# OnurBasci/TransformerBasedNavierStokeSolver

Hardware: AMD Instinct MI355X
Metric: ns64_train_samples_per_s (higher is better)
Workload: dtype f32

## Files before the change

transformerbasednavierstokesolver_amd/csrc/pa2d_gemm.hip:

```cpp
#include "pa2d_gemm_common.h"
#include <string.h>


static Pa2dEnv read_env() {
    auto is = [](const char* n, const char* pre) { const char* e = getenv(n); return e && strncmp(e, pre, strlen(pre)) == 0; };
    auto num = [](const char* n, int dflt) { const char* e = getenv(n); return (e && e[0]) ? atoi(e) : dflt; };
    Pa2dEnv v;
    v.conv_halo = is("PA2D_CONV_HALO", "o") ? 0 : (is("PA2D_CONV_HALO", "f") ? 2 : 1);
    v.mc_big_off = is("PA2D_MC_BIG", "o") ? 1 : 0;
    v.kc_bk16 = num("PA2D_KC_BK", 0) == 16 ? 1 : 0;
    v.mc_bk = num("PA2D_MC_BK", 16) == 32 ? 32 : 16;
    v.mc_splits = num("PA2D_MC_SPLITS", 0);
    v.mcb_splits = num("PA2D_MCB_SPLITS", 0);
    v.lin_dw_split = is("PA2D_LIN_DW_SPLIT", "of") ? 0 : 1;
    v.lin_panel = is("PA2D_LIN_PANEL", "of") ? 0 : 1;
    v.lin_rowpanel = is("PA2D_LIN_ROWPANEL", "of") ? 0 : 1;
    v.lin_small_split = is("PA2D_LIN_SMALL_SPLIT", "of") ? 0 : 1;
    v.conv_mfma16 = num("PA2D_CONV_MFMA", 16) == 32 ? 0 : 1;
    v.mc_mfma16 = num("PA2D_MC_MFMA", 16) == 32 ? 0 : 1;
    v.split_big = num("PA2D_SPLIT_BIG", 1);
    v.slice_map = is("PA2D_SLICE_MAP", "l") ? 0 : 1;
    v.default_engine = is("PA2D_GEMM", "f") ? 0 : (is("PA2D_GEMM", "b") ? 2 : 1);
    return v;
}
static Pa2dEnv g_env = read_env();
const Pa2dEnv& pa2d_env() { return g_env; }
static int kc_bk(bool im2col, int Cin) {
    if (im2col && pa2d_env().kc_bk16) return 16;
    return (!im2col || (Cin % 32) == 0) ? 32 : 16;
}
KCTile kc_tile(int M, int N, bool im2col, int Cin) {
    const int tiles_m = ceil_div(M, 128);
    const long long t128 = (long long)tiles_m * ceil_div(N, 128);
    const long long t12864 = (long long)tiles_m * ceil_div(N, 64);
    const int bk = kc_bk(im2col, Cin);
    if (N > 64 && t128 >= 384) return {128, 128, bk};
    if (t12864 >= 384 || M <= 64) return {128, 64, bk};
// ... 169 lines not shown

int pa2d_gemm_bwd_data(const float* dy, long long lddy, const float* w, long long ldw, const float* pre,
                       long long ldpre, int act, float* dx, long long lddx, const void* wimg, void* ws, size_t ws_bytes, int M,
                       int N, int K, int engine, hipStream_t st) {
    if (ldw != K) return PA2D_ERR_ARG;
    if (N & 3) return PA2D_ERR_ARG;
    if (M <= 0) return PA2D_OK;
    if (ws_bytes < (size_t)N * K * sizeof(float)) return PA2D_ERR_WORKSPACE;
    float* const wt_ws = (float*)ws;
    KCParams p = dense_bwd_data_params(dy, lddy, wt_ws, pre, ldpre, act, dx, lddx, M, N, K, engine, false);
    const size_t img = rowpanel_image_bytes(K, N, engine);
    if (img && wimg) p.wimg = const_cast<void*>(wimg);
    else if (img && ws_bytes >= (size_t)N * K * sizeof(float) + img) {
        p.wimg = (char*)ws + (size_t)N * K * sizeof(float); p.wsrc = w; p.wsn = 1; p.wsk = ldw;
    }
    if (!(p.wimg && rowpanel_applies(p) && (M % 128) == 0)) {
        const int rc = launch_repack(w, nullptr, wt_ws, 0, N, K, 0, 0, st);
        if (rc) return rc;
    }
    return launch_kc(p, false, st);
}

size_t pa2d_gemm_bwd_weight_workspace(int M, int N, int K, int engine) {
    (void)engine;
    const MCPlan pl = plan_mc(N, K, M);
    return (pl.slab_floats + (size_t)pl.splits * N) * sizeof(float);
}

int pa2d_gemm_bwd_weight(const float* dy, long long lddy, const float* x, long long ldx, float* dw, float* db,
                         void* ws, size_t ws_bytes, int M, int N, int K, int accumulate, int engine, hipStream_t st) {
    if (!engine_ok(engine)) return PA2D_ERR_ARG;
    if (M <= 0) {
        if (accumulate) return PA2D_OK;
        const int rz = pa2d_zero(dw, sizeof(float) * N * K, st);
        return rz ? rz : pa2d_zero(db, sizeof(float) * N, st);
    }
    if (ws_bytes < pa2d_gemm_bwd_weight_workspace(M, N, K, engine)) return PA2D_ERR_WORKSPACE;
    const MCPlan pl = plan_mc(N, K, M);
    float* cs = db ? (float*)ws + pl.slab_floats : nullptr;
    const bool bfk = (engine == 1 || engine == 2) && pl.big && mc_f32src_applies(N, K, M, lddy, ldx);
    int rc = bfk ? launch_mc_f32src(dy, lddy, N, x, ldx, K, M, (float*)ws, pl, engine == 2 ? 1 : 3, cs, st)
                 : launch_mc(dy, lddy, N, x, ldx, K, M, false, 0, 0, 0, (float*)ws, pl, engine, st, cs);
    if (rc) return rc;
    rc = launch_reduce((const float*)ws, pl.splits, (long long)N * K, dw, nullptr, 0, 0, 0, st, accumulate);
    if (rc) return rc;
    if (db) rc = launch_reduce(cs, pl.splits, N, db, nullptr, 0, 0, 0, st, accumulate);
    return rc;
}


int pa2d_gemm_bias_act_fwd_bf16(const void* x, long long ldx, const float* w, long long ldw, const float* bias,
                                const void* res, long long ldres, void* y, long long ldy, void* pre, long long ldpre,
                                int M, int N, int K, int act, hipStream_t st) {
    return launch_kc(dense_fwd_params(x, ldx, w, ldw, bias, res, ldres, y, ldy, pre, ldpre, M, N, K, act, 2, true), false, st);
}

int pa2d_gemm_bwd_data_bf16(const void* dy, long long lddy, const float* w, long long ldw, const void* pre,
                            long long ldpre, int act, void* dx, long long lddx, float* wt_ws, int M, int N, int K,
                            hipStream_t st) {
    if (ldw != K) return PA2D_ERR_ARG;
    if (N & 3) return PA2D_ERR_ARG;
    if (M <= 0) return PA2D_OK;
    int rc = launch_repack(w, nullptr, wt_ws, 0, N, K, 0, 0, st);
    if (rc) return rc;
    return launch_kc(dense_bwd_data_params(dy, lddy, wt_ws, pre, ldpre, act, dx, lddx, M, N, K, 2, true), false, st);
}

size_t pa2d_gemm_bwd_weight_workspace_bf16(int M, int N, int K) {
    const MCPlan pl = plan_mc_planes_big(N, K, M);
    size_t a = pl.slab_floats, b = (size_t)colsum_blocks(M) * N;
// ... 24 lines not shown
```

transformerbasednavierstokesolver_amd/csrc/pa2d_gemm_common.h:

```cpp
#pragma once
#include "pa2d_internal.h"
#include "pa2d_bf16_split.h"
#include <stdlib.h>

#define EPI_ACT 1
#define EPI_STORE_PRE 2
#define EPI_MUL_DACT 4

struct KCParams {
    const float* A; long long lda;
    const float* B; long long ldb;
    float* C; long long ldc;
    const float* bias;
    const float* bias2; int bias_split;
    int depth;
    const float* res; long long ldres;
    float* aux; long long ldaux;
    int M, N, K;
    int act, epi;
    int H, W, Cin;
    unsigned a_bytes, b_bytes;
    unsigned c_bytes, res_bytes, aux_bytes;
    int apre;
    int engine;
// ... 69 lines not shown
    } else if (p.epi == EPI_ACT && gelu && !has_res) {
        KC_EPI(false, false, true, false, ACT_GELU)
    } else if (p.epi == EPI_MUL_DACT && gelu && !has_res) {
        KC_EPI(false, false, false, true, ACT_GELU)
    } else {
        const bool sp = p.epi & EPI_STORE_PRE, ac = p.epi & EPI_ACT, da = p.epi & EPI_MUL_DACT;
        if (da) { if (has_res) { KC_EPI(true, false, false, true, -1) } else { KC_EPI(false, false, false, true, -1) } }
        else if (sp && ac) { if (has_res) { KC_EPI(true, true, true, false, -1) } else { KC_EPI(false, true, true, false, -1) } }
        else if (ac) { if (has_res) { KC_EPI(true, false, true, false, -1) } else { KC_EPI(false, false, true, false, -1) } }
        else { if (has_res) { KC_EPI(true, true, false, false, -1) } else { KC_EPI(false, true, false, false, -1) } }
    }
#undef KC_EPI
}

struct MCParams {
    const float* A; long long lda; int Mi;
    int depth;
    const float* B; long long ldb; int Nj;
    float* slab;
    int Mk, chunks_per_split, splits;
    int H, W, Cin;
    unsigned a_bytes, b_bytes;
    float* colsum;
};
struct MCPlan { int big; int splits; int chunks_per_split; size_t slab_floats; };
struct KCTile { int bm, bn, bk; };

static inline bool engine_ok(int e) { return e >= 0 && e <= 2; }
bool use_split(int engine, int N, bool im2col, int Cin);
KCTile kc_tile(int M, int N, bool im2col, int Cin);
int launch_kc(const KCParams& p_in, bool im2col, hipStream_t st, hipEvent_t ev0 = nullptr, hipEvent_t ev1 = nullptr);
int launch_repack(const float* w0, const float* w1, float* dst, int mode, int N, int K, int C, int Cin, hipStream_t st,
                  int taps = 9);
int launch_kc_f32(const KCParams& p, bool im2col, const KCTile& t, hipStream_t st);
int launch_kc_split(KCParams& p, bool im2col, hipStream_t st);
bool kc_split_small_applies(const KCParams& p, bool im2col);
int launch_kc_split_small(const KCParams& p, hipStream_t st);
size_t planes_bytes(long long rows, int C, int NT);
int launch_split_planes(const float* src, long long ld, void* dst, long long rows, int C, int NT, hipStream_t st);
int launch_repack_split(const float* w0, const float* w1, void* dst, int bwd, int NT, int C, int Cin, hipStream_t st,
                        int taps = 9);
bool panel_applies(const KCParams& p, bool im2col);
int launch_kc_panel(const KCParams& p, hipStream_t st);
size_t rowpanel_image_bytes(int N, int K, int engine);
bool rowpanel_applies(const KCParams& p);
int launch_pack_weight_image(const float* w, long long sn, long long sk, void* img, int N, int K, hipStream_t st);
int launch_kc_rowpanel(const KCParams& p, const void* img, hipStream_t st);
bool conv_halo_applies(const KCParams& p);
int launch_conv_halo(const KCParams& p, hipStream_t st);
MCPlan plan_mc(int Mi, int Nj, int Mk);
int launch_mc(const float* A, long long lda, int Mi, const float* B, long long ldb, int Nj, int Mk, bool im2col,
              int H, int W, int Cin, float* slab, const MCPlan& pl, int engine, hipStream_t st, float* colsum = nullptr,
              int taps = 9, int depth = 1);
int launch_reduce(const float* slab, int nslab, long long count, float* out, float* out2, int mode, int C, int Cin,
                  hipStream_t st, int accumulate = 0, int taps = 9);
int pa2d_launch_reduce(const float* slab, int nslab, long long count, float* out, hipStream_t st);
bool mc_planes_supported(int C, int Cin);
int launch_mc_planes(const void* PA, const void* PB, int C, int Cin, int Mk, int H, int W, float* slab,
                     const MCPlan& pl, int NT, hipStream_t st);
bool mc_planes_big_applies(int C, int Cin, int Mk);
MCPlan plan_mc_planes_big(int Mi, int Nj, int Mk);
int launch_mc_planes_big(const void* PA, const void* PB, int C, int Cin, int Mk, int H, int W, float* slab,
                         const MCPlan& pl, int NT, hipStream_t st);
int launch_mc_planes_big_raw(const void* PA, int Mi, const void* PB, int Cin, int taps, int Mk, int H, int W, float* slab,
                             const MCPlan& pl, int NT, hipStream_t st);
bool mc_f32src_applies(int Mi, int Nj, int Mk, long long lda, long long ldb);
int launch_mc_f32src(const float* A, long long lda, int Mi, const float* B, long long ldb, int Nj, int Mk, float* slab,
                     const MCPlan& pl, int NT, float* colsum, hipStream_t st);
int colsum_blocks(int M);
int launch_colsum_bf16(const void* X, long long ld, int M, int N, float* out, float* partial, hipStream_t st,
                       float* out2 = nullptr, int split = 0, int accumulate = 0);
int launch_colsum(const float* X, long long ld, int M, int N, float* out, float* partial, hipStream_t st,
                  float* out2 = nullptr, int split = 0, int accumulate = 0);
```

transformerbasednavierstokesolver_amd/csrc/pa2d_gemm_mc.hip:

```cpp
#include "pa2d_gemm_common.h"


template <int NT>
__device__ __forceinline__ void mc_split_elem(float v, bf16x8 (&pl)[NT], int e) {
    const __bf16 h = (__bf16)v;
    pl[0][e] = h;
    if constexpr (NT == 3) {
        const float r1 = v - (float)h;
        const __bf16 m = (__bf16)r1;
        pl[1][e] = m;
        pl[2][e] = (__bf16)(r1 - (float)m);
    }
}
template <int BM, int BN, bool IM2COL, int NT, int BK = 16, int TAPS = 9>
__global__ __launch_bounds__(256, 2) void gemm_mc_kernel(const MCParams p) {
    constexpr int WM = BM / 2, WN = BN / 2, TM = WM / 32, TN = WN / 32;
    constexpr int A_TPR = BM / 4, A_RPP = 256 / A_TPR, A_IT = BK / A_RPP;
    constexpr int B_TPR = BN / 4, B_RPP = 256 / B_TPR, B_IT = BK / B_RPP;
    static_assert(TM >= 1 && TN >= 1 && A_IT >= 1 && B_IT >= 1, "tile");
    __shared__ __attribute__((aligned(16))) float smem[2 * BK * (BM + BN)];
    float* const As = smem;
    float* const Bs = smem + 2 * BK * BM;

    const int tid = threadIdx.x, lane = tid & 63, wave = tid >> 6;
// ... 148 lines not shown
                    acc[i][j] = __builtin_amdgcn_mfma_f32_32x32x2f32(af[kk & 1][i], bf[kk & 1][j], acc[i][j], 0, 0, 0);
        }
        __builtin_amdgcn_sched_group_barrier(0x100, TM + TN, 0);
#pragma unroll
        for (int kk = 0; kk < BK / 2 - 1; ++kk) {
            __builtin_amdgcn_sched_group_barrier(0x100, TM + TN, 0);
            __builtin_amdgcn_sched_group_barrier(0x008, TM * TN, 0);
        }
        __builtin_amdgcn_sched_group_barrier(0x008, TM * TN, 0);
        }
        if (c + 1 < c_end) MC_STORE(buf ^ 1)
        __syncthreads();
    }
#undef MC_LOAD
#undef MC_STORE

    if (do_cs) {
        *reinterpret_cast<float4*>(smem + a_r * BM + a_c) = cs;
        __syncthreads();
        for (int c = tid; c < BM; c += 256) {
            float t = 0.f;
#pragma unroll
            for (int r = 0; r < A_RPP; ++r) t += smem[r * BM + c];
            if (ti * BM + c < p.Mi) p.colsum[(size_t)split * p.Mi + ti * BM + c] = t;
        }
    }
    float* out = p.slab + (size_t)split * p.Mi * p.Nj;
    const int col0 = tj * BN + wn * WN + (lane & 31);
    const int row0 = ti * BM + wm * WM + 4 * (lane >> 5);
#pragma unroll
    for (int j = 0; j < TN; ++j) {
        const int col = col0 + j * 32;
        if (col >= p.Nj) continue;
#pragma unroll
        for (int i = 0; i < TM; ++i)
#pragma unroll
            for (int r = 0; r < 16; ++r) {
                const int row = row0 + i * 32 + (r & 3) + 8 * (r >> 2);
                if (row < p.Mi) out[(size_t)row * p.Nj + col] = acc[i][j][r];
            }
    }
}


MCPlan plan_mc(int Mi, int Nj, int Mk) {
    MCPlan pl;
    if (Mk < 1) Mk = 1;
    pl.big = (Mi > 64 && Nj > 64) ? 1 : 0;
    const int bm = pl.big ? 128 : 64;
    const int tiles = ceil_div(Mi, bm) * ceil_div(Nj, bm);
// ... 39 lines not shown
        }
        for (; k < nslab; k += 4) s0 += p[(size_t)k * count];
    }
    red[ty][tx] = (s0 + s1) + (s2 + s3);
    __syncthreads();
    if (ty != 0 || idx >= count) return;
    const float s = ((red[0][tx] + red[1][tx]) + red[2][tx]) + red[3][tx];
    float* dst;
    if (mode == 0) {
        dst = out + idx;
    } else if (mode == 2) {
        dst = idx < C ? out + idx : out2 + (idx - C);
    } else {
        const int ci = (int)(idx % Cin);
        const int tap = (int)((idx / Cin) % TAPS);
        const int co = (int)(idx / ((long long)Cin * TAPS));
        dst = (co < C ? out : out2) + ((size_t)(co % C) * Cin + ci) * TAPS + tap;
    }
    *dst = accumulate ? *dst + s : s;
}

int launch_mc(const float* A, long long lda, int Mi, const float* B, long long ldb, int Nj, int Mk,
                     bool im2col, int H, int W, int Cin, float* slab, const MCPlan& pl, int engine, hipStream_t st,
                     float* colsum, int taps, int depth) {
    if ((Mi & 3) || (Nj & 3) || (lda & 3) || (ldb & 3)) return PA2D_ERR_ARG;
    if (im2col && (Cin & 3)) return PA2D_ERR_UNSUPPORTED;
    MCParams p;
    p.A = A; p.lda = lda; p.Mi = Mi; p.B = B; p.ldb = ldb; p.Nj = Nj; p.slab = slab; p.Mk = Mk;
    p.chunks_per_split = pl.chunks_per_split; p.splits = pl.splits; p.H = H; p.W = W; p.Cin = Cin;
    p.colsum = colsum;
    p.depth = depth;
    {
        const unsigned long long ab = ((unsigned long long)(Mk - 1) * lda + Mi) * 4ull;
        const unsigned long long bb = ((unsigned long long)(Mk - 1) * ldb + (im2col ? Cin : Nj)) * 4ull;
        if (ab >= 0xFFFFFFF0ull || bb >= 0xFFFFFFF0ull) return PA2D_ERR_UNSUPPORTED;
        p.a_bytes = (unsigned)ab;
        p.b_bytes = (unsigned)bb;
    }
    const int bm = pl.big ? 128 : 64;
    const dim3 grid(ceil_div(Mi, bm) * ceil_div(Nj, bm) * pl.splits);
    const bool bf = engine == 2;
    const int mc_bk = pa2d_env().mc_bk;
    if (im2col && taps == 27) {
        if (pl.big && !bf && mc_bk == 32 && (pl.chunks_per_split % 2) == 0)
            hipLaunchKernelGGL((gemm_mc_kernel<128, 128, true, 0, 32, 27>), grid, dim3(256), 0, st, p);
        else if (pl.big && engine == 1 && (Cin % 32) == 0)
            hipLaunchKernelGGL((gemm_mc_kernel<128, 128, true, 3, 16, 27>), grid, dim3(256), 0, st, p);
        else if (pl.big && bf)
            hipLaunchKernelGGL((gemm_mc_kernel<128, 128, true, 1, 16, 27>), grid, dim3(256), 0, st, p);
        else if (pl.big)
            hipLaunchKernelGGL((gemm_mc_kernel<128, 128, true, 0, 16, 27>), grid, dim3(256), 0, st, p);
        else
            hipLaunchKernelGGL((gemm_mc_kernel<64, 64, true, 0, 16, 27>), grid, dim3(256), 0, st, p);
        PA2D_CHECK_LAUNCH();
// ... 126 lines not shown
```

transformerbasednavierstokesolver_amd/csrc/pa2d_gemm_mc_planes.hip:

```cpp
#include "pa2d_gemm_common.h"
#include "pa2d_bf16_split.h"

struct MCPlanesParams {
    const void* PA; int chA;
    const void* PB; int chB;
    float* slab;
    int Mi, Nj, Mk, chunks_per_split, splits, H, W, Cin;
    unsigned a_bytes, b_bytes;
    int taps;
    long long lda, ldb;
    float* colsum;
};

__device__ __forceinline__ unsigned img_off(int row, int ch) {
    return 256u * row + 16u * (ch ^ (((row & 3) << 2) | ((row >> 2) & 3)));
}

template <int NT, int KS, bool F32SRC = false, bool MF16 = false>
__global__ __launch_bounds__(256, 2) void gemm_mc_planes_kernel(const MCPlanesParams p) {
    constexpr int PIMG = 4096;
    constexpr int STAGE = 2 * NT * KS * PIMG;
    constexpr int NP = 2 * NT * KS;
    __shared__ __attribute__((aligned(16))) unsigned char smem[(MF16 ? 3 : 2) * STAGE];

    const int tid = threadIdx.x, lane = tid & 63, wave = tid >> 6;
    const int tiles_i = (p.Mi + 127) / 128, tiles_j = (p.Nj + 127) / 128;
    int tj, ti, split;
    {
        const int tiles = tiles_i * tiles_j;
        if ((p.splits & 7) == 0) {
            const int xcd = blockIdx.x & 7, slot = blockIdx.x >> 3, q = p.splits >> 3;
            split = xcd * q + slot / tiles;
            const int t = slot % tiles;
            tj = t % tiles_j;
// ... 192 lines not shown
                MP16_MMA(ib, afc)
#pragma unroll
                for (int pl = 0; pl < NT; ++pl) afc[pl] = afn[pl];
            }
            __syncthreads();
            const int t = sp;
            sp = sr;
            sr = sq;
            sq = t;
        }
#undef MP16_CONVERT
#undef MP16_WRITE
#undef MP16_MMA
#undef MP16_FRAG
        if (do_cs) {
            float* sm = reinterpret_cast<float*>(smem);
#pragma unroll
            for (int e = 0; e < 8; ++e) sm[frow * 128 + fc8 * 8 + e] = cs[e];
            __syncthreads();
            if (tid < 128) {
                float t = 0.f;
#pragma unroll
                for (int r = 0; r < 16; ++r) t += sm[r * 128 + tid];
                if (ti * 128 + tid < p.Mi) p.colsum[(size_t)split * p.Mi + ti * 128 + tid] = t;
            }
        }
        float* out = p.slab + (size_t)split * p.Mi * p.Nj;
#pragma unroll
        for (int j = 0; j < 4; ++j) {
            const int col = tj * 128 + wn * 64 + j * 16 + 4 * kq;
#pragma unroll
            for (int ib = 0; ib < 4; ++ib) {
                const int row = ti * 128 + wm * 64 + ib * 16 + (lane & 15);
                if (row < p.Mi && col < p.Nj) *reinterpret_cast<f32x4*>(out + (size_t)row * p.Nj + col) = acc[ib][j];
            }
        }
        return;
    }

    f32x16 acc[2][2];
#pragma unroll
    for (int i = 0; i < 2; ++i)
#pragma unroll
        for (int j = 0; j < 2; ++j)
#pragma unroll
            for (int r = 0; r < 16; ++r) acc[i][j][r] = 0.f;

    const int g = lane >> 4, q4 = (lane & 15) >> 2, pq = lane & 3;
    unsigned fa[2][2], fb[2][2];
#pragma unroll
// ... 43 lines not shown
                    acc[i][j] = __builtin_amdgcn_mfma_f32_32x32x16_bf16(af[i][0], bf[j][2], acc[i][j], 0, 0, 0);
                    acc[i][j] = __builtin_amdgcn_mfma_f32_32x32x16_bf16(af[i][1], bf[j][0], acc[i][j], 0, 0, 0);
                    acc[i][j] = __builtin_amdgcn_mfma_f32_32x32x16_bf16(af[i][0], bf[j][1], acc[i][j], 0, 0, 0);
                }
                acc[i][j] = __builtin_amdgcn_mfma_f32_32x32x16_bf16(af[i][0], bf[j][0], acc[i][j], 0, 0, 0);
            }
        }
        if (c + KS < c_end) { MP_STORE(buf ^ 1) }
        __syncthreads();
    }
#undef MP_LOAD
#undef MP_STORE

    if constexpr (F32SRC) {
        if (do_cs) {
            float* sm = reinterpret_cast<float*>(smem);
#pragma unroll
            for (int e = 0; e < 8; ++e) sm[frow * 128 + fc8 * 8 + e] = cs[e];
            __syncthreads();
            if (tid < 128) {
                float t = 0.f;
#pragma unroll
                for (int r = 0; r < 16; ++r) t += sm[r * 128 + tid];
                if (ti * 128 + tid < p.Mi) p.colsum[(size_t)split * p.Mi + ti * 128 + tid] = t;
            }
        }
    }
    float* out = p.slab + (size_t)split * p.Mi * p.Nj;
    const int col0 = tj * 128 + wn * 64 + (lane & 31);
    const int row0 = ti * 128 + wm * 64 + 4 * (lane >> 5);
#pragma unroll
    for (int j = 0; j < 2; ++j)
#pragma unroll
        for (int i = 0; i < 2; ++i)
#pragma unroll
            for (int r = 0; r < 16; ++r) {
                const int row = row0 + i * 32 + (r & 3) + 8 * (r >> 2);
                if (!F32SRC || (row < p.Mi && col0 + j * 32 < p.Nj)) out[(size_t)row * p.Nj + col0 + j * 32] = acc[i][j][r];
            }
}

bool mc_planes_supported(int C, int Cin) { return (C % 64) == 0 && (Cin % 128) == 0; }

int launch_mc_planes(const void* PA, const void* PB, int C, int Cin, int Mk, int H, int W, float* slab,
                     const MCPlan& pl, int NT, hipStream_t st) {
    if (!mc_planes_supported(C, Cin) || !pl.big) return PA2D_ERR_UNSUPPORTED;
    MCPlanesParams p;
    p.PA = PA; p.chA = 2 * C / 32; p.PB = PB; p.chB = Cin / 32; p.slab = slab;
    p.Mi = 2 * C; p.Nj = 9 * Cin; p.Mk = Mk; p.chunks_per_split = pl.chunks_per_split; p.splits = pl.splits;
    p.H = H; p.W = W; p.Cin = Cin; p.taps = 9;
    const unsigned long long ab = (unsigned long long)Mk * p.chA * NT * 64, bb = (unsigned long long)Mk * p.chB * NT * 64;
    if (ab >= 0xFFFFFFF0ull || bb >= 0xFFFFFFF0ull) return PA2D_ERR_UNSUPPORTED;
    p.a_bytes = (unsigned)ab; p.b_bytes = (unsigned)bb;
    const dim3 grid((p.Mi / 128) * (p.Nj / 128) * pl.splits);
    if (NT == 3) hipLaunchKernelGGL((gemm_mc_planes_kernel<3, 1>), grid, dim3(256), 0, st, p);
    else hipLaunchKernelGGL((gemm_mc_planes_kernel<1, 4>), grid, dim3(256), 0, st, p);
    PA2D_CHECK_LAUNCH();
    return PA2D_OK;
}

template <int NT, int KS, bool MF16 = false>
__global__ __launch_bounds__(512, 1) void gemm_mc_planes_big_kernel(const MCPlanesParams p, const int per_xcd) {
    constexpr int PIMG = 8192;
    constexpr int STAGE = 2 * NT * KS * PIMG;
    constexpr int NP = (2 * NT * KS * 512) / 512;
    extern __shared__ __attribute__((aligned(16))) unsigned char smem[];

    const int tid = threadIdx.x, lane = tid & 63, wave = tid >> 6;
    const int tiles_i = (p.Mi + 255) / 256, tiles_j = (p.Nj + 255) / 256;
    const int tiles = tiles_i * tiles_j;
    const int lin = (blockIdx.x & 7) * per_xcd + (blockIdx.x >> 3);
    if ((int)(blockIdx.x >> 3) >= per_xcd || lin >= tiles * p.splits) return;
    const int split = lin / tiles, t_ = lin - split * tiles;
    const int ti = t_ / tiles_j, tj = t_ - ti * tiles_j;
    const int wm = wave >> 2, wn = wave & 3;
    const int total_chunks = (p.Mk + 15) / 16;
    const int c_begin = split * p.chunks_per_split;
    const int c_end = min(total_chunks, c_begin + p.chunks_per_split);
    const int HW = p.taps == 1 ? 1 : p.H * p.W;

    const __amdgpu_buffer_rsrc_t ra_rsrc = __builtin_amdgcn_make_buffer_rsrc(const_cast<void*>(p.PA), 0, p.a_bytes, 0x00020000);
    const __amdgpu_buffer_rsrc_t rb_rsrc = __builtin_amdgcn_make_buffer_rsrc(const_cast<void*>(p.PB), 0, p.b_bytes, 0x00020000);

    const int row16 = tid >> 5, cgrp = (tid & 31) >> 2, piece = tid & 3;
// ... 53 lines not shown
#pragma unroll
        for (int r = 0; r < 2; ++r) {
            const int row = 8 * (kq & 1) + 4 * r + q4;
            const unsigned swz = (unsigned)(((row & 3) << 2) | ((row >> 2) & 3));
            fa[r] = 512u * row + 16u * ((unsigned)(wm * 16 + (pq >> 1)) ^ swz) + 8u * (pq & 1);
            fb[r] = 512u * row + 16u * ((unsigned)(wn * 8 + (pq >> 1)) ^ swz) + 8u * (pq & 1);
        }
        typedef __attribute__((address_space(3))) s16x4 lds_s16x4;
#define MB16_FRAG(base_, t_, pl_)                                                                         \
    __builtin_bit_cast(bf16x8, __builtin_shufflevector(                                                   \
        __builtin_amdgcn_ds_read_tr16_b64_v4i16((lds_s16x4*)(smem + ((base_[0] ^ ((unsigned)(t_) << 5)) + (pl_) * PIMG))), \
        __builtin_amdgcn_ds_read_tr16_b64_v4i16((lds_s16x4*)(smem + ((base_[1] ^ ((unsigned)(t_) << 5)) + (pl_) * PIMG))), \
        0, 1, 2, 3, 4, 5, 6, 7))
#define MB16_MMA(ib_, AF)                                                                                 \
    _Pragma("unroll") for (int j = 0; j < 4; ++j) {        \
        acc[ib_][j] = __builtin_amdgcn_mfma_f32_16x16x32_bf16(xf[j][1], AF[1], acc[ib_][j], 0, 0, 0);     \
        acc[ib_][j] = __builtin_amdgcn_mfma_f32_16x16x32_bf16(xf[j][0], AF[2], acc[ib_][j], 0, 0, 0);     \
        acc[ib_][j] = __builtin_amdgcn_mfma_f32_16x16x32_bf16(xf[j][2], AF[0], acc[ib_][j], 0, 0, 0);     \
        acc[ib_][j] = __builtin_amdgcn_mfma_f32_16x16x32_bf16(xf[j][0], AF[1], acc[ib_][j], 0, 0, 0);     \
        acc[ib_][j] = __builtin_amdgcn_mfma_f32_16x16x32_bf16(xf[j][1], AF[0], acc[ib_][j], 0, 0, 0);     \
        acc[ib_][j] = __builtin_amdgcn_mfma_f32_16x16x32_bf16(xf[j][0], AF[0], acc[ib_][j], 0, 0, 0);     \
    }
        const int nst = c_end - c_begin, steps = (nst + 1) >> 1;
        if (nst > 0) {
            MB_LOAD(c_begin, rg0)
            MB_STORE(0, rg0)
            MB_LOAD(c_begin + 1, rg0)
            MB_STORE(1, rg0)
            if (steps > 1) MB_LOAD(c_begin + 2, rg0)
        }
        __syncthreads();
        int sp = 0, sq = 1, sr = 2;
        for (int k = 0; k < steps; ++k) {
            const unsigned lo = (unsigned)((kq >> 1) ? sq : sp) * (unsigned)STAGE;
            const unsigned ua[2] = {fa[0] + lo, fa[1] + lo};
            const unsigned ub[2] = {fb[0] + lo + NT * PIMG, fb[1] + lo + NT * PIMG};
            bf16x8 xf[4][NT];
#pragma unroll
            for (int j = 0; j < 4; ++j)
#pragma unroll
                for (int pl = 0; pl < NT; ++pl) xf[j][pl] = MB16_FRAG(ub, j, pl);
            bf16x8 afc[NT], afn[NT];
#pragma unroll
            for (int pl = 0; pl < NT; ++pl) afc[pl] = MB16_FRAG(ua, 0, pl);
#pragma unroll
            for (int ib = 0; ib < 8; ++ib) {
                if (ib < 7) {
#pragma unroll
                    for (int pl = 0; pl < NT; ++pl) afn[pl] = MB16_FRAG(ua, ib + 1, pl);
                }
                if (ib == 4) {
                    MB_STORE(sr, rg0)
                    MB_LOAD(c_begin + 2 * k + 3, rg0)
                }
                if (ib == 7) {
                    __syncthreads();
                    MB_STORE(sp, rg0)
                    MB_LOAD(c_begin + 2 * k + 4, rg0)
                }
                MB16_MMA(ib, afc)
#pragma unroll
                for (int pl = 0; pl < NT; ++pl) afc[pl] = afn[pl];
            }
            __syncthreads();
            const int t = sp;
            sp = sr;
            sr = sq;
            sq = t;
        }
#undef MB16_MMA
#undef MB16_FRAG
        float* out = p.slab + (size_t)split * p.Mi * p.Nj;
#pragma unroll
        for (int j = 0; j < 4; ++j) {
            const int col = tj * 256 + wn * 64 + j * 16 + 4 * kq;
            if (col >= p.Nj) continue;
#pragma unroll
            for (int ib = 0; ib < 8; ++ib) {
                const int row = ti * 256 + wm * 128 + ib * 16 + (lane & 15);
                if (row < p.Mi) *reinterpret_cast<f32x4*>(out + (size_t)row * p.Nj + col) = acc[ib][j];
            }
        }
        return;
    }

    f32x16 acc[4][2];
#pragma unroll
    for (int i = 0; i < 4; ++i)
#pragma unroll
        for (int j = 0; j < 2; ++j)
#pragma unroll
            for (int r = 0; r < 16; ++r) acc[i][j][r] = 0.f;

    const int g = lane >> 4, q4 = (lane & 15) >> 2, pq = lane & 3;
    unsigned fa[4][2], fb[2][2];
// ... 41 lines not shown
                }                                                                                         \
                acc[i][j] = __builtin_amdgcn_mfma_f32_32x32x16_bf16(af[i][0], bf[j][0], acc[i][j], 0, 0, 0); \
            }                                                                                             \
    }
    if (c_begin < c_end) {
        MB_LOAD(c_begin, rg0)
        MB_STORE(0, rg0)
        if (c_begin + KS < c_end) MB_LOAD(c_begin + KS, rg0)
    }
    __syncthreads();
    for (int c = c_begin; c < c_end; c += KS) {
        const int buf = ((c - c_begin) / KS) & 1;
        if (c + KS < c_end) {
            MB_STORE(buf ^ 1, rg0)
            if (c + 2 * KS < c_end) MB_LOAD(c + 2 * KS, rg0)
        }
        MB_COMPUTE(buf)
        __syncthreads();
    }
#undef MB_COMPUTE
#undef MB_LOAD
#undef MB_STORE

    float* out = p.slab + (size_t)split * p.Mi * p.Nj;
    const int col0 = tj * 256 + wn * 64 + (lane & 31);
    const int row0 = ti * 256 + wm * 128 + 4 * (lane >> 5);
#pragma unroll
    for (int j = 0; j < 2; ++j) {
        const int col = col0 + j * 32;
        if (col >= p.Nj) continue;
#pragma unroll
        for (int i = 0; i < 4; ++i)
#pragma unroll
            for (int r = 0; r < 16; ++r) {
                const int row = row0 + i * 32 + (r & 3) + 8 * (r >> 2);
                if (row < p.Mi) out[(size_t)row * p.Nj + col] = acc[i][j][r];
            }
    }
}

MCPlan plan_mc_planes_big(int Mi, int Nj, int Mk) {
    MCPlan pl;
    if (Mk < 1) Mk = 1;
    pl.big = 2;
    const int tiles = ceil_div(Mi, 256) * ceil_div(Nj, 256);
    const int total_chunks = ceil_div(Mk, 16);
    int splits = 256 / tiles;
// ... 4 lines not shown
    pl.chunks_per_split = ceil_div(total_chunks, splits);
    pl.splits = ceil_div(total_chunks, pl.chunks_per_split);
    pl.slab_floats = (size_t)pl.splits * Mi * Nj;
    return pl;
}

bool mc_planes_big_applies(int C, int Cin, int Mk) {
    if (pa2d_env().mc_big_off) return false;
    return (C % 16) == 0 && (Cin % 32) == 0 && 2 * C >= 256 && 9 * Cin >= 256 && Mk >= 16 * 8 * 4;
}

int launch_mc_planes_big(const void* PA, const void* PB, int C, int Cin, int Mk, int H, int W, float* slab,
                         const MCPlan& pl, int NT, hipStream_t st) {
    return launch_mc_planes_big_raw(PA, 2 * C, PB, Cin, 9, Mk, H, W, slab, pl, NT, st);
}

int launch_mc_planes_big_raw(const void* PA, int Mi, const void* PB, int Cin, int taps, int Mk, int H, int W, float* slab,
                             const MCPlan& pl, int NT, hipStream_t st) {
    if ((Mi & 31) || (Cin & 31) || (taps != 1 && taps != 9)) return PA2D_ERR_UNSUPPORTED;
    MCPlanesParams p;
    p.PA = PA; p.chA = Mi / 32; p.PB = PB; p.chB = Cin / 32; p.slab = slab;
    p.Mi = Mi; p.Nj = taps * Cin; p.Mk = Mk; p.chunks_per_split = pl.chunks_per_split; p.splits = pl.splits;
    p.H = H; p.W = W; p.Cin = Cin; p.taps = taps;
    const unsigned long long ab = (unsigned long long)Mk * p.chA * NT * 64, bb = (unsigned long long)Mk * p.chB * NT * 64;
    if (ab >= 0xFFFFFFF0ull || bb >= 0xFFFFFFF0ull) return PA2D_ERR_UNSUPPORTED;
    p.a_bytes = (unsigned)ab; p.b_bytes = (unsigned)bb;
    const int wgs = ceil_div(p.Mi, 256) * ceil_div(p.Nj, 256) * pl.splits;
    const int per_xcd = ceil_div(wgs, 8);
    const dim3 grid(per_xcd * 8);
    if (NT == 3 && pa2d_env().mc_mfma16 && (reinterpret_cast<uintptr_t>(slab) & 15) == 0) {
        const int smem = 3 * 2 * 3 * 1 * 8192;
        {
            hipError_t e = hipFuncSetAttribute(reinterpret_cast<const void*>(&gemm_mc_planes_big_kernel<3, 1, true>),
                                               hipFuncAttributeMaxDynamicSharedMemorySize, smem);
            if (e != hipSuccess) return (int)e;
        }
        hipLaunchKernelGGL((gemm_mc_planes_big_kernel<3, 1, true>), grid, dim3(512), smem, st, p, per_xcd);
    } else if (NT == 3) {
        const int smem = 2 * 2 * 3 * 1 * 8192;
        {
            hipError_t e = hipFuncSetAttribute(reinterpret_cast<const void*>(&gemm_mc_planes_big_kernel<3, 1>),
                                               hipFuncAttributeMaxDynamicSharedMemorySize, smem);
            if (e != hipSuccess) return (int)e;
        }
        hipLaunchKernelGGL((gemm_mc_planes_big_kernel<3, 1>), grid, dim3(512), smem, st, p, per_xcd);
    } else {
        const int smem = 2 * 2 * 1 * 4 * 8192;
        {
            hipError_t e = hipFuncSetAttribute(reinterpret_cast<const void*>(&gemm_mc_planes_big_kernel<1, 4>),
                                               hipFuncAttributeMaxDynamicSharedMemorySize, smem);
            if (e != hipSuccess) return (int)e;
        }
        hipLaunchKernelGGL((gemm_mc_planes_big_kernel<1, 4>), grid, dim3(512), smem, st, p, per_xcd);
    }
    PA2D_CHECK_LAUNCH();
    return PA2D_OK;
}

bool mc_f32src_applies(int Mi, int Nj, int Mk, long long lda, long long ldb) {
    return pa2d_env().lin_dw_split && (Mi % 8) == 0 && (Nj % 8) == 0 && Mi > 64 && Nj > 64 && Mk >= 16 * 8 * 16 && (lda % 4) == 0 && (ldb % 4) == 0;
}

int launch_mc_f32src(const float* A, long long lda, int Mi, const float* B, long long ldb, int Nj, int Mk, float* slab,
                     const MCPlan& pl, int NT, float* colsum, hipStream_t st) {
    if (!pl.big) return PA2D_ERR_UNSUPPORTED;
    MCPlanesParams p = {};
    p.PA = A; p.PB = B; p.slab = slab; p.lda = lda; p.ldb = ldb; p.colsum = colsum;
    p.Mi = Mi; p.Nj = Nj; p.Mk = Mk; p.chunks_per_split = pl.chunks_per_split; p.splits = pl.splits;
    p.H = 1; p.W = 1; p.Cin = Nj; p.taps = 1; p.chA = 0; p.chB = 0;
    const unsigned long long ab = ((unsigned long long)(Mk - 1) * lda + Mi) * 4ull, bb = ((unsigned long long)(Mk - 1) * ldb + Nj) * 4ull;
    if (ab >= 0xFFFFFFF0ull || bb >= 0xFFFFFFF0ull) return PA2D_ERR_UNSUPPORTED;
    p.a_bytes = (unsigned)ab; p.b_bytes = (unsigned)bb;
    const dim3 grid(ceil_div(Mi, 128) * ceil_div(Nj, 128) * pl.splits);
    if (NT == 3 && pa2d_env().mc_mfma16 && (Nj % 4) == 0 && (reinterpret_cast<uintptr_t>(slab) & 15) == 0)
        hipLaunchKernelGGL((gemm_mc_planes_kernel<3, 1, true, true>), grid, dim3(256), 0, st, p);
    else if (NT == 3) hipLaunchKernelGGL((gemm_mc_planes_kernel<3, 1, true>), grid, dim3(256), 0, st, p);
    else hipLaunchKernelGGL((gemm_mc_planes_kernel<1, 4, true>), grid, dim3(256), 0, st, p);
    PA2D_CHECK_LAUNCH();
    return PA2D_OK;
}
```

transformerbasednavierstokesolver_amd/csrc/pa2d_internal.h:

```cpp
#pragma once
#include <hip/hip_runtime.h>
#include <stdint.h>

typedef float f32x16 __attribute__((ext_vector_type(16)));
typedef float f32x4 __attribute__((ext_vector_type(4)));

#define PA2D_OK 0
#define PA2D_ERR_ARG 1001
#define PA2D_ERR_UNSUPPORTED 1002
#define PA2D_ERR_WORKSPACE 1003

#define PA2D_CHECK_LAUNCH()                         \
    do {                                            \
        hipError_t e__ = hipGetLastError();         \
        if (e__ != hipSuccess) return (int)e__;     \
    } while (0)

enum { ACT_NONE = 0, ACT_GELU = 1, ACT_TANH = 2, ACT_SIGMOID = 3, ACT_RELU = 4, ACT_SOFTPLUS = 5,
       ACT_ELU = 6, ACT_SILU = 7 };

__device__ __forceinline__ float normal_cdf(float x, float& e_out) {
#pragma clang fp contract(off)
    const float z = fabsf(x) * 0.70710678118654752440f;
    const float t = __builtin_amdgcn_rcpf(fmaf(0.3275911f, z, 1.0f));
// ... 74 lines not shown
    __builtin_amdgcn_raw_buffer_store_b32(__float_as_uint(v), r, voff, 0, 0);
}

__device__ __forceinline__ float2 buf_load2(__amdgpu_buffer_rsrc_t r, unsigned voff) {
    typedef unsigned int u32x2_ __attribute__((ext_vector_type(2)));
    const u32x2_ v = __builtin_amdgcn_raw_buffer_load_b64(r, voff, 0, 0);
    return make_float2(__uint_as_float(v.x), __uint_as_float(v.y));
}
__device__ __forceinline__ void buf_store4(__amdgpu_buffer_rsrc_t r, unsigned voff, float4 v) {
    u32x4 u = {__float_as_uint(v.x), __float_as_uint(v.y), __float_as_uint(v.z), __float_as_uint(v.w)};
    __builtin_amdgcn_raw_buffer_store_b128(u, r, voff, 0, 0);
}

#define PA2D_ACT_SAVE_DERIVATIVE_BIT 0x100

struct Pa2dEnv {
    int conv_halo;
    int mc_big_off;
    int kc_bk16;
    int mc_bk;
    int mc_splits;
    int mcb_splits;
    int lin_dw_split;
    int lin_panel;
    int conv_mfma16;
    int mc_mfma16;
    int lin_small_split;
    int lin_rowpanel;
    int split_big;
    int slice_map;
    int default_engine;
};
const Pa2dEnv& pa2d_env();

static inline int pa2d_zero(void* p, size_t bytes, hipStream_t st) {
    if (!p || !bytes) return PA2D_OK;
    return (int)hipMemsetAsync(p, 0, bytes, st);
}
static inline int ceil_div(int a, int b) { return (a + b - 1) / b; }
static inline long long ceil_div_ll(long long a, long long b) { return (a + b - 1) / b; }

struct ReduceSegs { int nseg; long long begin[5]; float* dst[4]; };
int pa2d_launch_reduce_segs(const float* slab, int nslab, long long count, const ReduceSegs& segs, int accumulate,
                            hipStream_t st);

typedef __bf16 bf16_t;
// ... 85 lines not shown
```

Baseline: 70.52.

## Add 256-tile f32-source weight-gradient GEMM path and fuse dw/db reduction

Adds a 256x256-tile variant of the big planes kernel that loads f32 activations directly, splits them into three bf16 planes in registers, and accumulates column sums for the bias gradient. Linear weight-gradient GEMMs with 128<N,K<=256 take this path by default. Split-K partial records now interleave dw and db with a shared stride, so one reduce launch produces both. This aims to cut redundant operand loads across 128-tile blocks and one reduction launch, at the cost of more register pressure, different split counts and a larger workspace.

```diff
diff --git a/transformerbasednavierstokesolver_amd/csrc/pa2d_gemm.hip b/transformerbasednavierstokesolver_amd/csrc/pa2d_gemm.hip
--- a/transformerbasednavierstokesolver_amd/csrc/pa2d_gemm.hip
+++ b/transformerbasednavierstokesolver_amd/csrc/pa2d_gemm.hip
@@ -13,6 +13,7 @@
     v.mc_splits = num("PA2D_MC_SPLITS", 0);
     v.mcb_splits = num("PA2D_MCB_SPLITS", 0);
     v.lin_dw_split = is("PA2D_LIN_DW_SPLIT", "of") ? 0 : 1;
+    v.lin_dw_tile = num("PA2D_LIN_DW_TILE", 256) == 128 ? 128 : 256;
     v.lin_panel = is("PA2D_LIN_PANEL", "of") ? 0 : 1;
     v.lin_rowpanel = is("PA2D_LIN_ROWPANEL", "of") ? 0 : 1;
     v.lin_small_split = is("PA2D_LIN_SMALL_SPLIT", "of") ? 0 : 1;
@@ -228,9 +229,13 @@
 }
 
 size_t pa2d_gemm_bwd_weight_workspace(int M, int N, int K, int engine) {
-    (void)engine;
     const MCPlan pl = plan_mc(N, K, M);
-    return (pl.slab_floats + (size_t)pl.splits * N) * sizeof(float);
+    size_t recs = (size_t)pl.splits;
+    if (engine == 1 && mc_f32src_big_applies(N, K, M, 4, 4)) {
+        const size_t big = (size_t)plan_mc_planes_big(N, K, M).splits;
+        if (big > recs) recs = big;
+    }
+    return recs * ((size_t)N * K + N) * sizeof(float);
 }
 
 int pa2d_gemm_bwd_weight(const float* dy, long long lddy, const float* x, long long ldx, float* dw, float* db,
@@ -242,16 +247,17 @@
         return rz ? rz : pa2d_zero(db, sizeof(float) * N, st);
     }
     if (ws_bytes < pa2d_gemm_bwd_weight_workspace(M, N, K, engine)) return PA2D_ERR_WORKSPACE;
-    const MCPlan pl = plan_mc(N, K, M);
-    float* cs = db ? (float*)ws + pl.slab_floats : nullptr;
+    if ((long long)N * K > 0x7fffffffll) return PA2D_ERR_UNSUPPORTED;
+    const bool big256 = engine == 1 && mc_f32src_big_applies(N, K, M, lddy, ldx) && (reinterpret_cast<uintptr_t>(ws) & 15) == 0;
+    const MCPlan pl = big256 ? plan_mc_planes_big(N, K, M) : plan_mc(N, K, M);
+    const long long rec = (long long)N * K + (db ? N : 0);
+    float* cs = db ? (float*)ws + (size_t)N * K : nullptr;
     const bool bfk = (engine == 1 || engine == 2) && pl.big && mc_f32src_applies(N, K, M, lddy, ldx);
-    int rc = bfk ? launch_mc_f32src(dy, lddy, N, x, ldx, K, M, (float*)ws, pl, engine == 2 ? 1 : 3, cs, st)
-                 : launch_mc(dy, lddy, N, x, ldx, K, M, false, 0, 0, 0, (float*)ws, pl, engine, st, cs);
-    if (rc) return rc;
-    rc = launch_reduce((const float*)ws, pl.splits, (long long)N * K, dw, nullptr, 0, 0, 0, st, accumulate);
-    if (rc) return rc;
-    if (db) rc = launch_reduce(cs, pl.splits, N, db, nullptr, 0, 0, 0, st, accumulate);
-    return rc;
+    int rc = big256 ? launch_mc_f32src_big(dy, lddy, N, x, ldx, K, M, (float*)ws, pl, cs, st, rec)
+             : bfk  ? launch_mc_f32src(dy, lddy, N, x, ldx, K, M, (float*)ws, pl, engine == 2 ? 1 : 3, cs, st, rec)
+                    : launch_mc(dy, lddy, N, x, ldx, K, M, false, 0, 0, 0, (float*)ws, pl, engine, st, cs, 9, 1, rec);
+    if (rc) return rc;
+    return launch_reduce((const float*)ws, pl.splits, rec, dw, db, db ? 2 : 0, N * K, 0, st, accumulate);
 }
 
 
diff --git a/transformerbasednavierstokesolver_amd/csrc/pa2d_gemm_common.h b/transformerbasednavierstokesolver_amd/csrc/pa2d_gemm_common.h
--- a/transformerbasednavierstokesolver_amd/csrc/pa2d_gemm_common.h
+++ b/transformerbasednavierstokesolver_amd/csrc/pa2d_gemm_common.h
@@ -115,6 +115,7 @@
     int H, W, Cin;
     unsigned a_bytes, b_bytes;
     float* colsum;
+    long long slab_stride, cs_stride;
 };
 struct MCPlan { int big; int splits; int chunks_per_split; size_t slab_floats; };
 struct KCTile { int bm, bn, bk; };
@@ -144,7 +145,7 @@
 MCPlan plan_mc(int Mi, int Nj, int Mk);
 int launch_mc(const float* A, long long lda, int Mi, const float* B, long long ldb, int Nj, int Mk, bool im2col,
               int H, int W, int Cin, float* slab, const MCPlan& pl, int engine, hipStream_t st, float* colsum = nullptr,
-              int taps = 9, int depth = 1);
+              int taps = 9, int depth = 1, long long rec_stride = 0);
 int launch_reduce(const float* slab, int nslab, long long count, float* out, float* out2, int mode, int C, int Cin,
                   hipStream_t st, int accumulate = 0, int taps = 9);
 int pa2d_launch_reduce(const float* slab, int nslab, long long count, float* out, hipStream_t st);
@@ -159,7 +160,10 @@
                              const MCPlan& pl, int NT, hipStream_t st);
 bool mc_f32src_applies(int Mi, int Nj, int Mk, long long lda, long long ldb);
 int launch_mc_f32src(const float* A, long long lda, int Mi, const float* B, long long ldb, int Nj, int Mk, float* slab,
-                     const MCPlan& pl, int NT, float* colsum, hipStream_t st);
+                     const MCPlan& pl, int NT, float* colsum, hipStream_t st, long long rec_stride = 0);
+bool mc_f32src_big_applies(int Mi, int Nj, int Mk, long long lda, long long ldb);
+int launch_mc_f32src_big(const float* A, long long lda, int Mi, const float* B, long long ldb, int Nj, int Mk, float* slab,
+                         const MCPlan& pl, float* colsum, hipStream_t st, long long rec_stride = 0);
 int colsum_blocks(int M);
 int launch_colsum_bf16(const void* X, long long ld, int M, int N, float* out, float* partial, hipStream_t st,
                        float* out2 = nullptr, int split = 0, int accumulate = 0);
diff --git a/transformerbasednavierstokesolver_amd/csrc/pa2d_gemm_mc.hip b/transformerbasednavierstokesolver_amd/csrc/pa2d_gemm_mc.hip
--- a/transformerbasednavierstokesolver_amd/csrc/pa2d_gemm_mc.hip
+++ b/transformerbasednavierstokesolver_amd/csrc/pa2d_gemm_mc.hip
@@ -194,10 +194,10 @@
             float t = 0.f;
 #pragma unroll
             for (int r = 0; r < A_RPP; ++r) t += smem[r * BM + c];
-            if (ti * BM + c < p.Mi) p.colsum[(size_t)split * p.Mi + ti * BM + c] = t;
-        }
-    }
-    float* out = p.slab + (size_t)split * p.Mi * p.Nj;
+            if (ti * BM + c < p.Mi) p.colsum[(size_t)split * p.cs_stride + ti * BM + c] = t;
+        }
+    }
+    float* out = p.slab + (size_t)split * p.slab_stride;
     const int col0 = tj * BN + wn * WN + (lane & 31);
     const int row0 = ti * BM + wm * WM + 4 * (lane >> 5);
 #pragma unroll
@@ -283,7 +283,7 @@
 
 int launch_mc(const float* A, long long lda, int Mi, const float* B, long long ldb, int Nj, int Mk,
                      bool im2col, int H, int W, int Cin, float* slab, const MCPlan& pl, int engine, hipStream_t st,
-                     float* colsum, int taps, int depth) {
+                     float* colsum, int taps, int depth, long long rec_stride) {
     if ((Mi & 3) || (Nj & 3) || (lda & 3) || (ldb & 3)) return PA2D_ERR_ARG;
     if (im2col && (Cin & 3)) return PA2D_ERR_UNSUPPORTED;
     MCParams p;
@@ -291,6 +291,8 @@
     p.chunks_per_split = pl.chunks_per_split; p.splits = pl.splits; p.H = H; p.W = W; p.Cin = Cin;
     p.colsum = colsum;
     p.depth = depth;
+    p.slab_stride = rec_stride ? rec_stride : (long long)Mi * Nj;
+    p.cs_stride = rec_stride ? rec_stride : Mi;
     {
         const unsigned long long ab = ((unsigned long long)(Mk - 1) * lda + Mi) * 4ull;
         const unsigned long long bb = ((unsigned long long)(Mk - 1) * ldb + (im2col ? Cin : Nj)) * 4ull;
diff --git a/transformerbasednavierstokesolver_amd/csrc/pa2d_gemm_mc_planes.hip b/transformerbasednavierstokesolver_amd/csrc/pa2d_gemm_mc_planes.hip
--- a/transformerbasednavierstokesolver_amd/csrc/pa2d_gemm_mc_planes.hip
+++ b/transformerbasednavierstokesolver_amd/csrc/pa2d_gemm_mc_planes.hip
@@ -10,6 +10,7 @@
     int taps;
     long long lda, ldb;
     float* colsum;
+    long long slab_stride, cs_stride;
 };
 
 __device__ __forceinline__ unsigned img_off(int row, int ch) {
@@ -248,10 +249,10 @@
                 float t = 0.f;
 #pragma unroll
                 for (int r = 0; r < 16; ++r) t += sm[r * 128 + tid];
-                if (ti * 128 + tid < p.Mi) p.colsum[(size_t)split * p.Mi + ti * 128 + tid] = t;
-            }
-        }
-        float* out = p.slab + (size_t)split * p.Mi * p.Nj;
+                if (ti * 128 + tid < p.Mi) p.colsum[(size_t)split * p.cs_stride + ti * 128 + tid] = t;
+            }
+        }
+        float* out = p.slab + (size_t)split * p.slab_stride;
 #pragma unroll
         for (int j = 0; j < 4; ++j) {
             const int col = tj * 128 + wn * 64 + j * 16 + 4 * kq;
@@ -341,11 +342,11 @@
                 float t = 0.f;
 #pragma unroll
                 for (int r = 0; r < 16; ++r) t += sm[r * 128 + tid];
-                if (ti * 128 + tid < p.Mi) p.colsum[(size_t)split * p.Mi + ti * 128 + tid] = t;
-            }
-        }
-    }
-    float* out = p.slab + (size_t)split * p.Mi * p.Nj;
+                if (ti * 128 + tid < p.Mi) p.colsum[(size_t)split * p.cs_stride + ti * 128 + tid] = t;
+            }
+        }
+    }
+    float* out = p.slab + (size_t)split * p.slab_stride;
     const int col0 = tj * 128 + wn * 64 + (lane & 31);
     const int row0 = ti * 128 + wm * 64 + 4 * (lane >> 5);
 #pragma unroll
@@ -368,6 +369,7 @@
     p.PA = PA; p.chA = 2 * C / 32; p.PB = PB; p.chB = Cin / 32; p.slab = slab;
     p.Mi = 2 * C; p.Nj = 9 * Cin; p.Mk = Mk; p.chunks_per_split = pl.chunks_per_split; p.splits = pl.splits;
     p.H = H; p.W = W; p.Cin = Cin; p.taps = 9;
+    p.colsum = nullptr; p.slab_stride = (long long)p.Mi * p.Nj; p.cs_stride = p.Mi;
     const unsigned long long ab = (unsigned long long)Mk * p.chA * NT * 64, bb = (unsigned long long)Mk * p.chB * NT * 64;
     if (ab >= 0xFFFFFFF0ull || bb >= 0xFFFFFFF0ull) return PA2D_ERR_UNSUPPORTED;
     p.a_bytes = (unsigned)ab; p.b_bytes = (unsigned)bb;
@@ -378,7 +380,7 @@
     return PA2D_OK;
 }
 
-template <int NT, int KS, bool MF16 = false>
+template <int NT, int KS, bool MF16 = false, bool F32SRC = false>
 __global__ __launch_bounds__(512, 1) void gemm_mc_planes_big_kernel(const MCPlanesParams p, const int per_xcd) {
     constexpr int PIMG = 8192;
     constexpr int STAGE = 2 * NT * KS * PIMG;
@@ -478,7 +480,57 @@
         acc[ib_][j] = __builtin_amdgcn_mfma_f32_16x16x32_bf16(xf[j][0], AF[0], acc[ib_][j], 0, 0, 0);     \
     }
         const int nst = c_end - c_begin, steps = (nst + 1) >> 1;
-        if (nst > 0) {
+        const int c8 = tid & 31;
+        const bool fok_a = ti * 256 + c8 * 8 < p.Mi, fok_b = tj * 256 + c8 * 8 < p.Nj;
+        const unsigned fcol_a = (unsigned)(ti * 256 + c8 * 8) * 4u, fcol_b = (unsigned)(tj * 256 + c8 * 8) * 4u;
+        const unsigned fpitch_a = (unsigned)p.lda * 4u, fpitch_b = (unsigned)p.ldb * 4u;
+        const bool do_cs = F32SRC && p.colsum != nullptr;
+        u32x4 rf[4];
+        bf16x8 pk[2][NT];
+        float cs[8];
+#pragma unroll
+        for (int e = 0; e < 8; ++e) cs[e] = 0.f;
+#define MBF_LOAD_OP(c_, op_)                                                         \
+    {                                                                                                     \
+        const int m_ = (c_) * 16 + row16;                                                                 \
+        const bool ok_ = m_ < p.Mk && (c_) < c_end && ((op_) ? fok_b : fok_a);                            \
+        const unsigned o_ = ok_ ? (unsigned)m_ * ((op_) ? fpitch_b : fpitch_a) + ((op_) ? fcol_b : fcol_a) : OOB_OFF; \
+        rf[(op_) * 2] = __builtin_amdgcn_raw_buffer_load_b128((op_) ? rb_rsrc : ra_rsrc, o_, 0, 0);       \
+        rf[(op_) * 2 + 1] = __builtin_amdgcn_raw_buffer_load_b128((op_) ? rb_rsrc : ra_rsrc, ok_ ? o_ + 16u : OOB_OFF, 0, 0); \
+    }
+#define MBF_LOAD(c_) MBF_LOAD_OP(c_, 0) MBF_LOAD_OP(c_, 1)
+#define MBF_CONVERT_OP(op)                                                                                \
+    {                                                                                                     \
+        const u32x4 u0_ = rf[op * 2], u1_ = rf[op * 2 + 1];                                               \
+        const float4 v0_ = make_float4(__uint_as_float(u0_.x), __uint_as_float(u0_.y), __uint_as_float(u0_.z), __uint_as_float(u0_.w)); \
+        const float4 v1_ = make_float4(__uint_as_float(u1_.x), __uint_as_float(u1_.y), __uint_as_float(u1_.z), __uint_as_float(u1_.w)); \
+        if (op == 0 && do_cs) {                                                                           \
+            cs[0] += v0_.x; cs[1] += v0_.y; cs[2] += v0_.z; cs[3] += v0_.w;                               \
+            cs[4] += v1_.x; cs[5] += v1_.y; cs[6] += v1_.z; cs[7] += v1_.w;                               \
+        }                                                                                                 \
+        bf16x4 h0_, m0_, l0_, h1_, m1_, l1_;                                                              \
+        split3(v0_, h0_, m0_, l0_);                                                                       \
+        split3(v1_, h1_, m1_, l1_);                                                                       \
+        pk[op][0] = __builtin_shufflevector(h0_, h1_, 0, 1, 2, 3, 4, 5, 6, 7);                            \
+        pk[op][1] = __builtin_shufflevector(m0_, m1_, 0, 1, 2, 3, 4, 5, 6, 7);                            \
+        pk[op][2] = __builtin_shufflevector(l0_, l1_, 0, 1, 2, 3, 4, 5, 6, 7);                            \
+    }
+#define MBF_WRITE_OP(buf_, op)                                                                            \
+    _Pragma("unroll") for (int pl = 0; pl < NT; ++pl)                                                     \
+        *reinterpret_cast<bf16x8*>(smem + (buf_) * STAGE + ((op) * NT + pl) * PIMG + lds_off) = pk[op][pl];
+#define MBF_CONVERT() MBF_CONVERT_OP(0) MBF_CONVERT_OP(1)
+#define MBF_WRITE(buf_) MBF_WRITE_OP(buf_, 0) MBF_WRITE_OP(buf_, 1)
+        if constexpr (F32SRC) {
+            if (nst > 0) {
+                MBF_LOAD(c_begin)
+                MBF_CONVERT()
+                MBF_WRITE(0)
+                MBF_LOAD(c_begin + 1)
+                MBF_CONVERT()
+                MBF_WRITE(1)
+                MBF_LOAD(c_begin + 2)
+            }
+        } else if (nst > 0) {
             MB_LOAD(c_begin, rg0)
             MB_STORE(0, rg0)
             MB_LOAD(c_begin + 1, rg0)
@@ -501,10 +553,36 @@
             for (int pl = 0; pl < NT; ++pl) afc[pl] = MB16_FRAG(ua, 0, pl);
 #pragma unroll
             for (int ib = 0; ib < 8; ++ib) {
-                if (ib < 7) {
+                if (ib < 7 && !(F32SRC && (ib == 3 || ib == 4))) {
 #pragma unroll
                     for (int pl = 0; pl < NT; ++pl) afn[pl] = MB16_FRAG(ua, ib + 1, pl);
                 }
+                if constexpr (F32SRC) {
+                    if (ib == 3) {
+                        __builtin_amdgcn_sched_barrier(0);
+                        MBF_CONVERT_OP(0)
+                        MBF_WRITE_OP(sr, 0)
+                        MBF_LOAD_OP(c_begin + 2 * k + 3, 0)
+                        __builtin_amdgcn_sched_barrier(0);
+                    }
+                    if (ib == 4) {
+                        __builtin_amdgcn_sched_barrier(0);
+                        MBF_CONVERT_OP(1)
+                        MBF_WRITE_OP(sr, 1)
+                        MBF_LOAD_OP(c_begin + 2 * k + 3, 1)
+                        __builtin_amdgcn_sched_barrier(0);
+                    }
+                    if (ib == 7) {
+                        MBF_CONVERT()
+                        __syncthreads();
+                        MBF_WRITE(sp)
+                        MBF_LOAD(c_begin + 2 * k + 4)
+                    }
+                    if (ib == 3 || ib == 4) {
+#pragma unroll
+                        for (int pl = 0; pl < NT; ++pl) afn[pl] = MB16_FRAG(ua, ib + 1, pl);
+                    }
+                } else {
                 if (ib == 4) {
                     MB_STORE(sr, rg0)
                     MB_LOAD(c_begin + 2 * k + 3, rg0)
@@ -514,6 +592,7 @@
                     MB_STORE(sp, rg0)
                     MB_LOAD(c_begin + 2 * k + 4, rg0)
                 }
+                }
                 MB16_MMA(ib, afc)
 #pragma unroll
                 for (int pl = 0; pl < NT; ++pl) afc[pl] = afn[pl];
@@ -526,7 +605,25 @@
         }
 #undef MB16_MMA
 #undef MB16_FRAG
-        float* out = p.slab + (size_t)split * p.Mi * p.Nj;
+#undef MBF_LOAD
+#undef MBF_LOAD_OP
+#undef MBF_CONVERT
+#undef MBF_CONVERT_OP
+#undef MBF_WRITE
+#undef MBF_WRITE_OP
+        if (do_cs) {
+            float* sm = reinterpret_cast<float*>(smem);
+#pragma unroll
+            for (int e = 0; e < 8; ++e) sm[row16 * 256 + c8 * 8 + e] = cs[e];
+            __syncthreads();
+            if (tid < 256) {
+                float t = 0.f;
+#pragma unroll
+                for (int r = 0; r < 16; ++r) t += sm[r * 256 + tid];
+                if (ti * 256 + tid < p.Mi) p.colsum[(size_t)split * p.cs_stride + ti * 256 + tid] = t;
+            }
+        }
+        float* out = p.slab + (size_t)split * p.slab_stride;
 #pragma unroll
         for (int j = 0; j < 4; ++j) {
             const int col = tj * 256 + wn * 64 + j * 16 + 4 * kq;
@@ -614,7 +711,7 @@
 #undef MB_LOAD
 #undef MB_STORE
 
-    float* out = p.slab + (size_t)split * p.Mi * p.Nj;
+    float* out = p.slab + (size_t)split * p.slab_stride;
     const int col0 = tj * 256 + wn * 64 + (lane & 31);
     const int row0 = ti * 256 + wm * 128 + 4 * (lane >> 5);
 #pragma unroll
@@ -665,6 +762,7 @@
     p.PA = PA; p.chA = Mi / 32; p.PB = PB; p.chB = Cin / 32; p.slab = slab;
     p.Mi = Mi; p.Nj = taps * Cin; p.Mk = Mk; p.chunks_per_split = pl.chunks_per_split; p.splits = pl.splits;
     p.H = H; p.W = W; p.Cin = Cin; p.taps = taps;
+    p.colsum = nullptr; p.slab_stride = (long long)p.Mi * p.Nj; p.cs_stride = p.Mi;
     const unsigned long long ab = (unsigned long long)Mk * p.chA * NT * 64, bb = (unsigned long long)Mk * p.chB * NT * 64;
     if (ab >= 0xFFFFFFF0ull || bb >= 0xFFFFFFF0ull) return PA2D_ERR_UNSUPPORTED;
     p.a_bytes = (unsigned)ab; p.b_bytes = (unsigned)bb;
@@ -704,21 +802,53 @@
     return pa2d_env().lin_dw_split && (Mi % 8) == 0 && (Nj % 8) == 0 && Mi > 64 && Nj > 64 && Mk >= 16 * 8 * 16 && (lda % 4) == 0 && (ldb % 4) == 0;
 }
 
-int launch_mc_f32src(const float* A, long long lda, int Mi, const float* B, long long ldb, int Nj, int Mk, float* slab,
-                     const MCPlan& pl, int NT, float* colsum, hipStream_t st) {
-    if (!pl.big) return PA2D_ERR_UNSUPPORTED;
-    MCPlanesParams p = {};
+static int f32src_params(MCPlanesParams& p, const float* A, long long lda, int Mi, const float* B, long long ldb, int Nj, int Mk,
+                         float* slab, const MCPlan& pl, float* colsum, long long rec_stride) {
+    p = {};
     p.PA = A; p.PB = B; p.slab = slab; p.lda = lda; p.ldb = ldb; p.colsum = colsum;
+    p.slab_stride = rec_stride ? rec_stride : (long long)Mi * Nj;
+    p.cs_stride = rec_stride ? rec_stride : Mi;
     p.Mi = Mi; p.Nj = Nj; p.Mk = Mk; p.chunks_per_split = pl.chunks_per_split; p.splits = pl.splits;
     p.H = 1; p.W = 1; p.Cin = Nj; p.taps = 1; p.chA = 0; p.chB = 0;
     const unsigned long long ab = ((unsigned long long)(Mk - 1) * lda + Mi) * 4ull, bb = ((unsigned long long)(Mk - 1) * ldb + Nj) * 4ull;
     if (ab >= 0xFFFFFFF0ull || bb >= 0xFFFFFFF0ull) return PA2D_ERR_UNSUPPORTED;
     p.a_bytes = (unsigned)ab; p.b_bytes = (unsigned)bb;
+    return PA2D_OK;
+}
+
+int launch_mc_f32src(const float* A, long long lda, int Mi, const float* B, long long ldb, int Nj, int Mk, float* slab,
+                     const MCPlan& pl, int NT, float* colsum, hipStream_t st, long long rec_stride) {
+    if (pl.big != 1) return PA2D_ERR_UNSUPPORTED;
+    MCPlanesParams p;
+    const int rp = f32src_params(p, A, lda, Mi, B, ldb, Nj, Mk, slab, pl, colsum, rec_stride);
+    if (rp) return rp;
     const dim3 grid(ceil_div(Mi, 128) * ceil_div(Nj, 128) * pl.splits);
-    if (NT == 3 && pa2d_env().mc_mfma16 && (Nj % 4) == 0 && (reinterpret_cast<uintptr_t>(slab) & 15) == 0)
+    if (NT == 3 && pa2d_env().mc_mfma16 && (Nj % 4) == 0 && (p.slab_stride % 4) == 0 && (reinterpret_cast<uintptr_t>(slab) & 15) == 0)
         hipLaunchKernelGGL((gemm_mc_planes_kernel<3, 1, true, true>), grid, dim3(256), 0, st, p);
     else if (NT == 3) hipLaunchKernelGGL((gemm_mc_planes_kernel<3, 1, true>), grid, dim3(256), 0, st, p);
     else hipLaunchKernelGGL((gemm_mc_planes_kernel<1, 4, true>), grid, dim3(256), 0, st, p);
     PA2D_CHECK_LAUNCH();
     return PA2D_OK;
 }
+
+bool mc_f32src_big_applies(int Mi, int Nj, int Mk, long long lda, long long ldb) {
+    return pa2d_env().lin_dw_tile == 256 && pa2d_env().mc_mfma16 && mc_f32src_applies(Mi, Nj, Mk, lda, ldb) && Mi > 128 &&
+           Mi <= 256 && Nj > 128 && Nj <= 256 && (Mi % 32) == 0 && (Nj % 32) == 0;
+}
+
+int launch_mc_f32src_big(const float* A, long long lda, int Mi, const float* B, long long ldb, int Nj, int Mk, float* slab,
+                         const MCPlan& pl, float* colsum, hipStream_t st, long long rec_stride) {
+    if (pl.big != 2 || Mi > 256 || Nj > 256 || (Mi & 31) || (Nj & 31)) return PA2D_ERR_UNSUPPORTED;
+    if ((reinterpret_cast<uintptr_t>(slab) & 15) || (rec_stride & 3)) return PA2D_ERR_ARG;
+    MCPlanesParams p;
+    const int rp = f32src_params(p, A, lda, Mi, B, ldb, Nj, Mk, slab, pl, colsum, rec_stride);
+    if (rp) return rp;
+    const int per_xcd = ceil_div(pl.splits, 8);
+    const int smem = 3 * 2 * 3 * 1 * 8192;
+    const hipError_t e = hipFuncSetAttribute(reinterpret_cast<const void*>(&gemm_mc_planes_big_kernel<3, 1, true, true>),
+                                             hipFuncAttributeMaxDynamicSharedMemorySize, smem);
+    if (e != hipSuccess) return (int)e;
+    hipLaunchKernelGGL((gemm_mc_planes_big_kernel<3, 1, true, true>), dim3(per_xcd * 8), dim3(512), smem, st, p, per_xcd);
+    PA2D_CHECK_LAUNCH();
+    return PA2D_OK;
+}
diff --git a/transformerbasednavierstokesolver_amd/csrc/pa2d_internal.h b/transformerbasednavierstokesolver_amd/csrc/pa2d_internal.h
--- a/transformerbasednavierstokesolver_amd/csrc/pa2d_internal.h
+++ b/transformerbasednavierstokesolver_amd/csrc/pa2d_internal.h
@@ -120,6 +120,7 @@
     int mc_splits;
     int mcb_splits;
     int lin_dw_split;
+    int lin_dw_tile;
     int lin_panel;
     int conv_mfma16;
     int mc_mfma16;
```

New measurement: 71.17 (median of 6 runs). Within noise of the previous version (+0.9%).
